# IIT-PAVIS/DiffAssemble

Measured on AMD Instinct MI355X. Metric: denoising steps/sec (900-piece dense graph, T=100), higher is better.
Workload: dtype bf16

## Files before the change

### diffassemble_amd/csrc/da_gemm_xpanel.hip

```cpp
#include <stdlib.h>

#include "da_gemm_common.h"

namespace da {

typedef __attribute__((ext_vector_type(16))) float f32x16p;

__device__ __forceinline__ void xp_dma16(unsigned lds_addr, unsigned voff, const void *sbase) {
    asm volatile("s_mov_b32 m0, %0\n\ts_nop 0\n\tglobal_load_lds_dwordx4 %1, %2" ::"s"(lds_addr), "v"(voff), "s"(sbase) : "memory");
}
__device__ __forceinline__ void xp_dma4(unsigned lds_addr, unsigned voff, const void *sbase) {
    asm volatile("s_mov_b32 m0, %0\n\ts_nop 0\n\tglobal_load_lds_dword %1, %2" ::"s"(lds_addr), "v"(voff), "s"(sbase) : "memory");
}

__host__ __device__ __forceinline__ int xp_pi(int m) { return 16 * ((m >> 2) & 1) + 4 * (m >> 3) + (m & 3); }

__global__ void k_pack_w_xpanel(int Nout, int K, int ldw, const bf16_t *W, u32x4 *Wp) {
    const int KS = K / 16;
    const size_t i = (size_t)blockIdx.x * blockDim.x + threadIdx.x;
    const size_t total = (size_t)((Nout + 255) / 256) * 8 * KS * 64;
    if (i >= total) return;
    const int lane = (int)(i & 63), s = (int)((i >> 6) % KS);
    const int gw = (int)((i >> 6) / KS);
    const int col = gw * 32 + xp_pi(lane & 31);
    u32x4 v = {0u, 0u, 0u, 0u};
    if (col < Nout) v = *(const u32x4 *)(W + (size_t)col * ldw + 16 * s + 8 * (lane >> 5));
    Wp[i] = v;
}

size_t xpanel_packed_bytes(int K, int Nout) { return (size_t)((Nout + 255) / 256) * 256 * (size_t)K * 2; }

int pack_w_xpanel(int K, int Nout, const void *W, int ldw, void *packed, hipStream_t st) {
    if (ldw <= 0) ldw = K;
    const size_t total = xpanel_packed_bytes(K, Nout) / 16;
    k_pack_w_xpanel<<<(unsigned)((total + 255) / 256), 256, 0, st>>>(Nout, K, ldw, (const bf16_t *)W, (u32x4 *)packed);
    DA_LAUNCH_CHECK();
    return 0;
}

template <int U> __device__ __forceinline__ void xp_store_rot(bf16_t *dst, u32x4 o0, u32x4 o1);
#define DA_XP_STORE_ROT(U, R0, R1)                                                                                        \
    template <> __device__ __forceinline__ void xp_store_rot<U>(bf16_t * dst, u32x4 o0, u32x4 o1) {                       \
        asm volatile("global_store_dwordx4 %0, %1, off\n\tglobal_store_dwordx4 %0, %2, off offset:16" ::"v"(dst), R0(o0), R1(o1) : "memory"); \
    }
DA_XP_STORE_ROT(0, "{v[224:227]}", "{v[228:231]}")
DA_XP_STORE_ROT(1, "{v[232:235]}", "{v[236:239]}")
DA_XP_STORE_ROT(2, "{v[240:243]}", "{v[244:247]}")
DA_XP_STORE_ROT(3, "{v[248:251]}", "{v[252:255]}")
#undef DA_XP_STORE_ROT
template <int U> struct XpSlot { static constexpr int value = U; };

template <int KIN, bool QKV, int ACT>
__global__ __launch_bounds__(512) void k_gemm_xpanel(GemmParams p, const u32x4 *__restrict__ Wp, int T, int ncg) {
    constexpr int KS = KIN / 16;
    constexpr int ROWB = KIN * 2;
    constexpr int TILEB = 32 * ROWB;
    constexpr int NDMA = TILEB / 1024;
    constexpr int CPR = ROWB / 16;
    extern __shared__ __attribute__((aligned(16))) unsigned char smem[];
    unsigned char *panel = smem;
    unsigned char *slots = smem + T * TILEB;
    float *bias_s = (float *)(slots + T * 128);
    const int tid = threadIdx.x, lane = tid & 63;
    const int wid = __builtin_amdgcn_readfirstlane(tid >> 6);
    const int nrt = (p.M + 31) >> 5;
    const int t0 = blockIdx.x * T;
    const int ntile = min(T, nrt - t0);
    if (ntile <= 0) return;
    const int i32 = lane & 31, half = lane >> 5;

    u32x4 wA[KS], wB[KS];
    const unsigned wlane = (unsigned)lane * 16u;
    auto load_w = [&](u32x4 (&wf)[KS], int g) {
        const char *src = (const char *)(Wp + ((size_t)(g * 8 + wid) * KS) * 64);
#pragma unroll
        for (int s = 0; s < KS; ++s)
            asm volatile("global_load_dwordx4 %0, %1, %2" : "=v"(wf[s]) : "v"(wlane), "s"(src + s * 1024) : "memory");
    };
    load_w(wA, 0);
    {
        const int rsub = lane / CPR, pc = lane % CPR;
        const unsigned panel_lds = (unsigned)(size_t)panel, slots_lds = (unsigned)(size_t)slots;
        for (int t = wid; t < ntile; t += 8) {
            const int row0 = (t0 + t) * 32;
            const char *base = (const char *)p.A + (size_t)row0 * (size_t)p.lda * 2;
            const int rmax = p.M - 1 - row0;
#pragma unroll
            for (int q = 0; q < NDMA; ++q) {
                const int row = q * (64 / CPR) + rsub;
                const int lc = pc ^ (row & 15);
                xp_dma16(panel_lds + t * TILEB + q * 1024, (unsigned)min(row, rmax) * (unsigned)p.lda * 2u + (unsigned)lc * 16u, base);
            }
            if (QKV && lane < 32) xp_dma4(slots_lds + t * 128, (unsigned)min(lane, rmax) * 4u, p.row_map + row0);
        }
        for (int c = tid; c < ncg * 256; c += 512) bias_s[c] = (p.bias && c < p.Nout) ? p.bias[c] : 0.f;
        asm volatile("s_waitcnt vmcnt(0)" ::: "memory");
        __syncthreads();
    }
    if (ncg > 1) load_w(wB, 1);

    auto run_group = [&](u32x4 (&wf)[KS], int g) {
        const int col0 = g * 256 + wid * 32;
        const bool active = col0 < p.Nout;
        const int colc = col0 + 16 * half;
        f32x16p bzv;
#pragma unroll
        for (int e = 0; e < 4; ++e) {
            const f32x4 b = *(const f32x4 *)(bias_s + colc + 4 * e);
            bzv[4 * e] = b[0]; bzv[4 * e + 1] = b[1]; bzv[4 * e + 2] = b[2]; bzv[4 * e + 3] = b[3];
        }
        bf16_t *dbase;
        size_t rstride;
        bool use_slot = false;
        if (!QKV) {
            dbase = (bf16_t *)p.out + colc;
            rstride = (size_t)p.ldo;
        } else {
            const int which = min(colc / p.HC, 3), f = colc - which * p.HC;
            if (which == 2 && p.Cv > 0) {
                const int h = f / p.Cv, c = f - h * p.Cv;
                dbase = (bf16_t *)p.Vt + (size_t)h * p.n_pad * p.Cv + c;
                rstride = (size_t)p.Cv;
                use_slot = true;
            } else if (which == 3) {
                dbase = (bf16_t *)p.S + f;
                rstride = (size_t)p.HC;
            } else {
                const int h = f / p.C, c = f - h * p.C;
                dbase = (bf16_t *)(which == 0 ? p.Q : (which == 1 ? p.Kb : p.Vt)) + (size_t)h * p.n_pad * p.C + c;
                rstride = (size_t)p.C;
                use_slot = true;
            }
        }
        auto tile_body = [&](int t, auto slot) {
            const unsigned char *buf = panel + t * TILEB + i32 * ROWB;
            f32x16p acc;
#pragma unroll
            for (int r = 0; r < 16; ++r) acc[r] = 0.f;
            constexpr int PF = 4, NG = KS / PF;
            u32x4 xa[2][PF];
#pragma unroll
            for (int s = 0; s < PF; ++s) xa[0][s] = *(const u32x4 *)(buf + (((2 * s + half) ^ (i32 & 15)) << 4));
#pragma unroll
            for (int gq = 0; gq < NG; ++gq) {
                if (gq + 1 < NG) {
#pragma unroll
                    for (int s = 0; s < PF; ++s)
                        xa[(gq + 1) & 1][s] = *(const u32x4 *)(buf + (((2 * ((gq + 1) * PF + s) + half) ^ (i32 & 15)) << 4));
                }
                __builtin_amdgcn_sched_barrier(0);
#pragma unroll
                for (int s = 0; s < PF; ++s)
                    acc = __builtin_amdgcn_mfma_f32_32x32x16_bf16(__builtin_bit_cast(bf16x8, wf[gq * PF + s]),
                                                                  __builtin_bit_cast(bf16x8, xa[gq & 1][s]), acc, 0, 0, 0);
                __builtin_amdgcn_sched_barrier(0);
            }
            bf16x8 o0, o1;
#pragma unroll
            for (int e = 0; e < 8; ++e) {
                o0[e] = (__bf16)apply_act(acc[e] + bzv[e], ACT);
                o1[e] = (__bf16)apply_act(acc[8 + e] + bzv[8 + e], ACT);
            }
            const bool lastt = t == ntile - 1;
            if (lastt) {
                asm volatile("s_waitcnt vmcnt(0)" ::: "memory");
            }
            const int m = (t0 + t) * 32 + i32;
            if (active && m < p.M && !(p.debug & 256)) {
                const size_t ridx = use_slot ? (size_t)((const int32_t *)(slots + t * 128))[i32] : (size_t)m;
                bf16_t *dst = dbase + ridx * rstride;
                xp_store_rot<decltype(slot)::value>(dst, __builtin_bit_cast(u32x4, o0), __builtin_bit_cast(u32x4, o1));
            }
        };
        for (int t = 0; t < ntile; t += 4) {
            tile_body(t, XpSlot<0>());
            if (t + 1 < ntile) tile_body(t + 1, XpSlot<1>());
            if (t + 2 < ntile) tile_body(t + 2, XpSlot<2>());
            if (t + 3 < ntile) tile_body(t + 3, XpSlot<3>());
        }
        __builtin_amdgcn_sched_barrier(0);
        if (g + 2 < ncg) load_w(wf, g + 2);
        __builtin_amdgcn_sched_barrier(0);
    };
    for (int g = 0; g < ncg; g += 2) {
        run_group(wA, g);
        if (g + 1 < ncg) run_group(wB, g + 1);
    }
}

int xpanel_mode() {
    const int v = cfg().xpanel;
    if (v >= 0) return v ? 1 : 0;
    const bool other = DA_XENV_SET("DA_DISABLE_WREG") || DA_XENV_SET("DA_WREG2") || DA_XENV_SET("DA_WREG_DIRECT") || DA_XENV_SET("DA_DISABLE_ASTAT") ||
                       DA_XENV_SET("DA_GEMM_DEBUG") || DA_XENV_SET("DA_GEMM_PROF_PTR") || DA_XENV_SET("DA_GEMM_THIN");
    return other ? 0 : 2;
}
bool xpanel_in_model() { return xpanel_mode() != 0; }

int launch_gemm_xpanel(int prec, const GemmParams &p0, const QkvScatter *qs, int act, const void *wpacked, hipStream_t st) {
    if (prec != DA_PREC_BF16 || !wpacked) return -1;
    GemmParams p = p0;
    if ((p.K != 128 && p.K != 256) || p.pre || p.res || (p.Nout & 31) || p.Nout < 512 || p.Nout > 4096) return -1;
    if (qs) {
        if ((qs->HC & 15) || (qs->C & 15) || (qs->Cv & 15) || act != DA_ACT_NONE) return -1;
    } else if ((p.ldo & 7) || (((size_t)p.out) & 15)) {
        return -1;
    }
    const int nrt = (p.M + 31) / 32;
    const int ncg = (p.Nout + 255) / 256;
    const int tileb = 32 * p.K * 2;
    const int tmax = (160 * 1024 - ncg * 1024 - 512) / (tileb + 128);
    int T = (nrt + 255) / 256;
    if (T > tmax) T = tmax;
    if (T < 4) return -1;
    const int nwg = (nrt + T - 1) / T;
    const int lds = T * (tileb + 128) + ncg * 1024;
#define DA_XP(KK, QQ, AA)                                                                                                 \
    do {                                                                                                                  \
        static bool attr = false;                                                                                         \
        if (!attr) {                                                                                                      \
            DA_CHECK_HIP(hipFuncSetAttribute((const void *)k_gemm_xpanel<KK, QQ, AA>, hipFuncAttributeMaxDynamicSharedMemorySize, 160 * 1024)); \
            attr = true;                                                                                                  \
        }                                                                                                                 \
        k_gemm_xpanel<KK, QQ, AA><<<nwg, 512, lds, st>>>(p, (const u32x4 *)wpacked, T, ncg);                              \
    } while (0)
    if (qs) {
        if (p.K == 256) DA_XP(256, true, DA_ACT_NONE); else DA_XP(128, true, DA_ACT_NONE);
    } else if (act == DA_ACT_GELU) {
        if (p.K == 256) DA_XP(256, false, DA_ACT_GELU); else DA_XP(128, false, DA_ACT_GELU);
    } else if (act == DA_ACT_NONE) {
        if (p.K == 256) DA_XP(256, false, DA_ACT_NONE); else DA_XP(128, false, DA_ACT_NONE);
    } else {
        return -1;
    }
#undef DA_XP
    DA_LAUNCH_CHECK();
    return 0;
}

}
```

Baseline: 99340.

## Add register-resident-weight GEMM variant splitting output columns across workgroups

Adds k_gemm_xres, a GEMM kernel where each workgroup keeps two 256-column weight blocks resident in registers and streams a panel of A row-tiles from LDS. Work is split over row panels and column slices, with an XCD-aware block index remap and a cost-based planner that chooses the panel size. By default it is used for non-QKV GEMMs when the planned cost is not worse than the existing cross-panel kernel. This is meant to raise parallelism and cut per-workgroup weight streaming. In exchange, A panels are reloaded once per column slice.

```diff
diff --git a/diffassemble_amd/csrc/da_gemm_xpanel.hip b/diffassemble_amd/csrc/da_gemm_xpanel.hip
--- a/diffassemble_amd/csrc/da_gemm_xpanel.hip
+++ b/diffassemble_amd/csrc/da_gemm_xpanel.hip
@@ -188,6 +188,170 @@
     }
 }
 
+constexpr int XR_NB = 2;
+
+template <int KIN, bool QKV, int ACT>
+__global__ __launch_bounds__(512) void k_gemm_xres(GemmParams p, const u32x4 *__restrict__ Wp, int T, int nslice, int nwg, int per, int ncg) {
+    constexpr int KS = KIN / 16;
+    constexpr int ROWB = KIN * 2;
+    constexpr int TILEB = 32 * ROWB;
+    constexpr int NDMA = TILEB / 1024;
+    constexpr int CPR = ROWB / 16;
+    extern __shared__ __attribute__((aligned(16))) unsigned char smem[];
+    unsigned char *panel = smem;
+    unsigned char *slots = smem + T * TILEB;
+    float *bias_s = (float *)(slots + T * 128);
+    const int tid = threadIdx.x, lane = tid & 63;
+    const int wid = __builtin_amdgcn_readfirstlane(tid >> 6);
+    const int v = (int)(blockIdx.x & 7) * per + (int)(blockIdx.x >> 3);
+    if (v >= nwg) return;
+    const int pnl = v / nslice, slice = v - pnl * nslice;
+    const int nrt = (p.M + 31) >> 5;
+    const int t0 = pnl * T;
+    const int ntile = min(T, nrt - t0);
+    if (ntile <= 0) return;
+    const int g0 = slice * XR_NB;
+    const int nb = min(XR_NB, ncg - g0);
+    const int i32 = lane & 31, half = lane >> 5;
+
+    u32x4 wf[XR_NB][KS];
+    {
+        const unsigned wlane = (unsigned)lane * 16u;
+#pragma unroll
+        for (int b = 0; b < XR_NB; ++b) {
+            if (b < nb) {
+                const char *src = (const char *)(Wp + ((size_t)((g0 + b) * 8 + wid) * KS) * 64);
+#pragma unroll
+                for (int s = 0; s < KS; ++s)
+                    asm volatile("global_load_dwordx4 %0, %1, %2" : "=v"(wf[b][s]) : "v"(wlane), "s"(src + s * 1024) : "memory");
+            }
+        }
+    }
+    {
+        const int rsub = lane / CPR, pc = lane % CPR;
+        const unsigned panel_lds = (unsigned)(size_t)panel, slots_lds = (unsigned)(size_t)slots;
+        for (int t = wid; t < ntile; t += 8) {
+            const int row0 = (t0 + t) * 32;
+            const char *base = (const char *)p.A + (size_t)row0 * (size_t)p.lda * 2;
+            const int rmax = p.M - 1 - row0;
+#pragma unroll
+            for (int q = 0; q < NDMA; ++q) {
+                const int row = q * (64 / CPR) + rsub;
+                const int lc = pc ^ (row & 15);
+                xp_dma16(panel_lds + t * TILEB + q * 1024, (unsigned)min(row, rmax) * (unsigned)p.lda * 2u + (unsigned)lc * 16u, base);
+            }
+            if (QKV && lane < 32) xp_dma4(slots_lds + t * 128, (unsigned)min(lane, rmax) * 4u, p.row_map + row0);
+        }
+        for (int c = tid; c < XR_NB * 256; c += 512) {
+            const int col = g0 * 256 + c;
+            bias_s[c] = (p.bias && col < p.Nout) ? p.bias[col] : 0.f;
+        }
+        asm volatile("s_waitcnt vmcnt(0)" ::: "memory");
+        __syncthreads();
+    }
+    if (p.debug & 1024) return;
+
+    bf16_t *dbase[XR_NB];
+    int rstride[XR_NB];
+    bool use_slot[XR_NB], active[XR_NB];
+#pragma unroll
+    for (int b = 0; b < XR_NB; ++b) {
+        const int col0 = (g0 + b) * 256 + wid * 32;
+        active[b] = b < nb && col0 < p.Nout;
+        const int colc = col0 + 16 * half;
+        use_slot[b] = false;
+        if (!QKV) {
+            dbase[b] = (bf16_t *)p.out + colc;
+            rstride[b] = p.ldo;
+        } else {
+            const int which = min(colc / p.HC, 3), f = colc - which * p.HC;
+            if (which == 2 && p.Cv > 0) {
+                const int h = f / p.Cv, c = f - h * p.Cv;
+                dbase[b] = (bf16_t *)p.Vt + (size_t)h * p.n_pad * p.Cv + c;
+                rstride[b] = p.Cv;
+                use_slot[b] = true;
+            } else if (which == 3) {
+                dbase[b] = (bf16_t *)p.S + f;
+                rstride[b] = p.HC;
+            } else {
+                const int h = f / p.C, c = f - h * p.C;
+                dbase[b] = (bf16_t *)(which == 0 ? p.Q : (which == 1 ? p.Kb : p.Vt)) + (size_t)h * p.n_pad * p.C + c;
+                rstride[b] = p.C;
+                use_slot[b] = true;
+            }
+        }
+    }
+    const bool do_store = !(p.debug & 256);
+
+    auto tile_body = [&](int t, auto u0) {
+        constexpr int U0 = decltype(u0)::value;
+        const unsigned char *buf = panel + t * TILEB + i32 * ROWB;
+        f32x16p acc[XR_NB];
+#pragma unroll
+        for (int b = 0; b < XR_NB; ++b)
+#pragma unroll
+            for (int r = 0; r < 16; ++r) acc[b][r] = 0.f;
+        constexpr int PF = 4, NG = KS / PF;
+        u32x4 xa[2][PF];
+#pragma unroll
+        for (int s = 0; s < PF; ++s) xa[0][s] = *(const u32x4 *)(buf + (((2 * s + half) ^ (i32 & 15)) << 4));
+#pragma unroll
+        for (int gq = 0; gq < NG; ++gq) {
+            if (gq + 1 < NG) {
+#pragma unroll
+                for (int s = 0; s < PF; ++s)
+                    xa[(gq + 1) & 1][s] = *(const u32x4 *)(buf + (((2 * ((gq + 1) * PF + s) + half) ^ (i32 & 15)) << 4));
+            }
+            __builtin_amdgcn_sched_barrier(0);
+#pragma unroll
+            for (int s = 0; s < PF; ++s)
+#pragma unroll
+                for (int b = 0; b < XR_NB; ++b)
+                    acc[b] = __builtin_amdgcn_mfma_f32_32x32x16_bf16(__builtin_bit_cast(bf16x8, wf[b][gq * PF + s]),
+                                                                     __builtin_bit_cast(bf16x8, xa[gq & 1][s]), acc[b], 0, 0, 0);
+            __builtin_amdgcn_sched_barrier(0);
+        }
+        const int m = (t0 + t) * 32 + i32;
+        const size_t slot_row = QKV ? (size_t)((const int32_t *)(slots + t * 128))[i32] : (size_t)m;
+        auto epilogue = [&](auto bc) {
+            constexpr int b = decltype(bc)::value;
+            const float *bz = bias_s + b * 256 + wid * 32 + 16 * half;
+            bf16x8 o0, o1;
+#pragma unroll
+            for (int e4 = 0; e4 < 2; ++e4) {
+                const f32x4 ba = *(const f32x4 *)(bz + 4 * e4), bb = *(const f32x4 *)(bz + 8 + 4 * e4);
+#pragma unroll
+                for (int e = 0; e < 4; ++e) {
+                    o0[4 * e4 + e] = (__bf16)apply_act(acc[b][4 * e4 + e] + ba[e], ACT);
+                    o1[4 * e4 + e] = (__bf16)apply_act(acc[b][8 + 4 * e4 + e] + bb[e], ACT);
+                }
+            }
+            if (active[b] && m < p.M && do_store) {
+                bf16_t *dst = dbase[b] + (use_slot[b] ? slot_row : (size_t)m) * (size_t)rstride[b];
+                xp_store_rot<U0 + b>(dst, __builtin_bit_cast(u32x4, o0), __builtin_bit_cast(u32x4, o1));
+            }
+        };
+        static_assert(XR_NB == 2, "the epilogue below stores two column blocks");
+        epilogue(XpSlot<0>());
+        epilogue(XpSlot<1>());
+    };
+    for (int t = 0; t < ntile; t += 2) {
+        tile_body(t, XpSlot<0>());
+        if (t + 1 < ntile) tile_body(t + 1, XpSlot<2>());
+    }
+}
+
+static int xres_plan(int nrt, int nslice, int tmax, int *per_out, int *nwg_out) {
+    int best = 0, best_cost = 0;
+    for (int T = 4; T <= tmax; ++T) {
+        const int nwg = ((nrt + T - 1) / T) * nslice;
+        const int per = (nwg + 7) / 8;
+        const int cost = ((per + 31) / 32) * (T + 1);
+        if (!best || cost <= best_cost) { best = T; best_cost = cost; *per_out = per; *nwg_out = nwg; }
+    }
+    return best;
+}
+
 int xpanel_mode() {
     const int v = cfg().xpanel;
     if (v >= 0) return v ? 1 : 0;
@@ -214,6 +378,36 @@
     if (T > tmax) T = tmax;
     if (T < 4) return -1;
     const int nwg = (nrt + T - 1) / T;
+    const int xres_mode = DA_XENV("DA_XPANEL_RES", -1);
+    if (xres_mode == 1 || (xres_mode < 0 && !qs)) {
+        const int nslice = (ncg + XR_NB - 1) / XR_NB;
+        int per = 0, nwgr = 0;
+        const int TR = xres_plan(nrt, nslice, (160 * 1024 - XR_NB * 1024) / (tileb + 128), &per, &nwgr);
+        if (TR > 0 && ((per + 31) / 32) * TR * XR_NB <= ((nwg + 255) / 256) * T * ncg) {
+            const int ldsr = TR * (tileb + 128) + XR_NB * 1024;
+#define DA_XR(KK, QQ, AA)                                                                                                 \
+    do {                                                                                                                  \
+        static bool attr = false;                                                                                         \
+        if (!attr) {                                                                                                      \
+            DA_CHECK_HIP(hipFuncSetAttribute((const void *)k_gemm_xres<KK, QQ, AA>, hipFuncAttributeMaxDynamicSharedMemorySize, 160 * 1024)); \
+            attr = true;                                                                                                  \
+        }                                                                                                                 \
+        k_gemm_xres<KK, QQ, AA><<<8 * per, 512, ldsr, st>>>(p, (const u32x4 *)wpacked, TR, nslice, nwgr, per, ncg);      \
+    } while (0)
+            if (qs) {
+                if (p.K == 256) DA_XR(256, true, DA_ACT_NONE); else DA_XR(128, true, DA_ACT_NONE);
+            } else if (act == DA_ACT_GELU) {
+                if (p.K == 256) DA_XR(256, false, DA_ACT_GELU); else DA_XR(128, false, DA_ACT_GELU);
+            } else if (act == DA_ACT_NONE) {
+                if (p.K == 256) DA_XR(256, false, DA_ACT_NONE); else DA_XR(128, false, DA_ACT_NONE);
+            } else {
+                return -1;
+            }
+#undef DA_XR
+            DA_LAUNCH_CHECK();
+            return 0;
+        }
+    }
     const int lds = T * (tileb + 128) + ncg * 1024;
 #define DA_XP(KK, QQ, AA)                                                                                                 \
     do {                                                                                                                  \
```

New measurement: 99240, median of 3. Within noise of the previous version (-0.1%).
